# FrankBoesing/Minimal-SDR

Hardware: AMD Instinct MI355X
Metric: Msamples/s through IF->I/Q->FIR->demod->IIR chain; achieved HBM GB/s vs peak (higher is better)
Workload: dtype f32 (fp32 accumulate; matrix-core operands as 2 x fp16 pieces: int16 samples exact, taps 22 bits)

## Files before the change

### include/msdr.h

```cpp
#ifndef MSDR_H
#define MSDR_H

#include <stddef.h>
#include <stdint.h>

#ifdef __cplusplus
extern "C" {
#endif

#define MSDR_VERSION_MAJOR 0
#define MSDR_VERSION_MINOR 1

typedef int16_t q15_t;
typedef float float32_t;

typedef enum {
    MSDR_STATUS_SUCCESS        = 0,
    MSDR_STATUS_ARGUMENT_ERROR = -1,
    MSDR_STATUS_LENGTH_ERROR   = -2,
    MSDR_STATUS_SIZE_MISMATCH  = -3,
    MSDR_STATUS_NO_DEVICE      = -100,
    MSDR_STATUS_HIP_ERROR      = -101,
    MSDR_STATUS_OUT_OF_MEMORY  = -102
} msdr_status;
// ... 233 lines not shown
#define MSDR_FLAVOUR_SSB_UNITS    0x0001u
#define MSDR_FLAVOUR_ENV_UNITS    0x0002u
#define MSDR_FLAVOUR_SSB_FOLD     0x0004u
#define MSDR_FLAVOUR_ENV_FOLD     0x0008u
#define MSDR_FLAVOUR_FULL_RATE    0x0010u
#define MSDR_FLAVOUR_COMPACT      0x0020u
#define MSDR_FLAVOUR_SHARED_IQ    0x0040u
#define MSDR_FLAVOUR_AMTR         0x0080u
#define MSDR_FLAVOUR_BLOCK        0x0100u
#define MSDR_FLAVOUR_VALU_FOLD    0x0200u
#define MSDR_FLAVOUR_SEQ_CASCADE  0x0400u
#define MSDR_FLAVOUR_SEGMENTED    0x0800u
#define MSDR_FLAVOUR_FOLD_PERIOD_SHIFT 12
#define MSDR_FLAVOUR_FOLD_PERIOD(f) (((f) >> MSDR_FLAVOUR_FOLD_PERIOD_SHIFT) & 7u)
enum { MSDR_FLAVOUR_TAPS_PC = 0x8000u };
enum { MSDR_FLAVOUR_CASCADE_PC = 0x10000u };
enum { MSDR_FLAVOUR_OSC_PC = 0x20000u };
enum { MSDR_FLAVOUR_SHARED_IF = 0x40000u };
enum { MSDR_FLAVOUR_NCO_PC = 0x80000u };
enum { MSDR_FLAVOUR_DECIMATED = 0x100000u };
enum { MSDR_FLAVOUR_METER = 0x200000u };
enum { MSDR_FLAVOUR_IQ_OUT = 0x400000u };
int msdr_chain_get_info(msdr_chain *chain, msdr_chain_info *info);
const char *msdr_chain_node_kernel(msdr_chain *chain);
const char *msdr_biquad_q15_last_kernel(msdr_biquad_q15 *S);
const char *msdr_frontend_last_kernel(msdr_frontend *fe);
int msdr_chain_get_fir_history(msdr_chain *chain, uint32_t channel, int16_t *hist, uint32_t capacity, uint32_t *hist_len);
int msdr_chain_get_cmsis_state(msdr_chain *chain, uint32_t channel, float32_t *pState);
int msdr_chain_enable_timing(msdr_chain *chain, int on);
int msdr_chain_get_kernel_time(msdr_chain *chain, double *total_ms, uint64_t *launches, int reset);


typedef struct msdr_chain_graph msdr_chain_graph;
int msdr_chain_graph_create(msdr_chain *chain, uint32_t ticks, const int16_t *const *d_if, void *const *d_audio, uint64_t n_samples, msdr_chain_graph **out);
int msdr_chain_graph_launch(msdr_chain_graph *graph);
int msdr_chain_graph_destroy(msdr_chain_graph *graph);

#ifdef __cplusplus
}
#endif
#endif
```

### minimal-sdr_amd/csrc/msdr_api.hip

```cpp
#include <dlfcn.h>
#include "../../include/msdr.h"
#include "msdr_kernels.hiph"
#include "msdr_chain_fold.hiph"
#include <type_traits>
#include "msdr_chain_mfma.hiph"
#include "msdr_chain_mfw.hiph"
#include "msdr_frontend.hiph"
#include "msdr_spectrum.hiph"
#include "msdr_chain_q15mf.hiph"
#include "msdr_fir_f32mf.hiph"
#include "msdr_fir_f32tr.hiph"
#include "msdr_fir_f32tq.hiph"
#include "msdr_chain_amtr.hiph"
#include "msdr_chain_mfb.hiph"
#include "msdr_chain_q15mb.hiph"
#include "msdr_chain_q15pc.hiph"
#include "msdr_chain_f32pc.hiph"
#include "msdr_chain_oscpc.hiph"
#include "msdr_block.h"
#include "msdr_nco.h"
#include "msdr_design.h"
#include "msdr_cascade_state.h"
#include "msdr_kstack.h"
#include "msdr_sparse24.h"
// ... 2175 lines not shown
    float in_scale;
    uint32_t nstages;
    uint32_t nnodes;
    uint32_t time_segments, warmup_cfg;
    double pole_radius;
    void *d_taps, *d_osc;
    int *d_mode, *d_tapset;
    int16_t *d_hist[2];
    int cur;
    long long phase;
    BiquadCascadeTables<kChainR> *d_bq;
    float *d_bq_state;
    int fold_P;
    int mf_P;
    bool fold_fs4_exact;
    float *d_ftaps;
    int *d_fset;
    BiquadCascadeTables<kFoldR> *d_bq_fold;
    std::vector<int> h_mode, h_tapset;
    bool mf_ok;
    int mf_halo, mf_bsteps, mf_stride;
    int mf_xsteps = 0;
    int mf_merged[2] = {0, 0};
    char *d_mf_tab;
    BiquadCascadeTables<kMfL> *d_bq_mf;
    BiquadCascadeTables<32> *d_bq_mf32;
    uint32_t flags;
    int mfw_nw, mfw_waves_per_cu;
    char *d_at_tab; int at_ns, at_stride, at_nw;
    bool mf_compact, mf_share_iq;
    bool mf_fr;
    float *d_bq_state_alt;
    float *d_mw_iir;
    bool mfw_ssb_fold, mfw_am_fold;
    int mfw_am_rowlocal;
    uint32_t units_wgs_ssb;
    long long part_nseg[2], part_seg_len[2];
    long long units_tiles;
    int *d_units;
    size_t units_cap;
    uint64_t mode_gen, units_mode_gen;
    long long units_nseg;
    uint32_t units_wgs;
    int *d_btiles = nullptr;
    size_t btiles_cap = 0;
    uint64_t btiles_mode_gen = 0;
// ... 770 lines not shown
            }
        }
        if (ok && bsteps > 0) {
            const int stride = kMfHdrBytes + (bsteps + xsteps) * 2048;
            std::vector<char> blob((size_t)stride * tabs.size(), 0);
            for (size_t t = 0; t < tabs.size(); t++) {
                memcpy(blob.data() + t * stride, &tabs[t].h, sizeof(MfmaTableHeader));
                memcpy(blob.data() + t * stride + kMfHdrBytes, tabs[t].frags.data(), tabs[t].frags.size() * sizeof(_Float16));
            }
            rc = upload(ctx, blob, &c->d_mf_tab);
            if (!rc) {
                std::vector<BiquadCascadeTables<kMfL>> bt(1);
                make_cascade_tables<kMfL>(cfg->biquad_coeffs, (int)c->nstages, &bt[0]);
                rc = upload(ctx, bt, &c->d_bq_mf);
            }
            if (!rc) {
                std::vector<BiquadCascadeTables<32>> bt(1);
                make_cascade_tables<32>(cfg->biquad_coeffs, (int)c->nstages, &bt[0]);
                rc = upload(ctx, bt, &c->d_bq_mf32);
            }
            if (!rc) {
                c->mf_ok = true; c->mf_halo = H; c->mf_bsteps = bsteps; c->mf_stride = stride; c->mf_compact = compact;
                c->mf_xsteps = xsteps; c->mf_merged[0] = merged_min[0]; c->mf_merged[1] = merged_min[1];
                int best = 0, best_eff = 0, wcap = 16;
#ifdef MSDR_STAMPS
                if (const char *e = getenv("MSDR_DBG_NW")) wcap = std::max(1, std::min(16, atoi(e)));
#endif
                for (int w = 1; w <= wcap; w++) {
                    const size_t l = mw_lds_bytes(H, bsteps + xsteps, w, fr);
                    if (l > 160 * 1024) break;
                    const int wgs = std::min<int>((int)((160 * 1024) / l), wcap / w);
                    const int on_cu = wgs * w, eff = on_cu >= 4 ? 4 * (on_cu / 4) : on_cu;
                    if (eff > best_eff) { best_eff = eff; best = on_cu; c->mfw_nw = w; }
                }
                if (const char *e = getenv("MSDR_MFW_NW")) {
                    const int w = atoi(e);
                    if (w >= 1 && w <= 16 && mw_lds_bytes(H, bsteps + xsteps, w, fr) <= 160 * 1024) { c->mfw_nw = w; best = w * std::max<int>(1, std::min<int>((int)((160 * 1024) / mw_lds_bytes(H, bsteps + xsteps, w, fr)), 16 / w)); }
                }
                c->mfw_waves_per_cu = best;
                if (best > 0) rc = dzalloc(ctx, (size_t)c->channels * kBqStateFloats, &c->d_bq_state_alt);
                if (!rc && iirfold && !iirc.empty()) rc = upload(ctx, iirc, &c->d_mw_iir);
                c->mfw_ssb_fold = iirfold && !compact && c->d_mw_iir; c->mfw_am_fold = amfold && c->d_mw_iir;
                c->mfw_am_rowlocal = c->mfw_am_fold ? am_rowlocal : 0;
                if (best <= 0) c->mf_ok = false;
                if (fr && c->mfw_nw < 2) c->mf_ok = false;
            }
// ... 462 lines not shown
            const long long rounds = (nch * ns + slots - 1) / slots;
            const double cost = (double)rounds * (double)(st + (ns > 1 ? t.warm_tiles : 0));
            if (cost < best * 0.999) { best = cost; ns_ = ns; }
        }
    } else {
        long long min_seg_tiles = std::max<long long>(4, 32 * t.warm_tiles);
        long long max_nseg = std::max<long long>(1, t.tiles / min_seg_tiles);
        long long want = c->time_segments > 1 ? c->time_segments : std::max<long long>(1, (2048 + nch - 1) / nch);
        ns_ = std::max<long long>(1, std::min(want, max_nseg));
    }
    const long long st = (t.tiles + ns_ - 1) / ns_;
    return (t.tiles + st - 1) / st;
}

struct ChainLaunch {
    const char *kname;
    unsigned grid, block;
    size_t lds_bytes;
    long long nseg;
    int tile;
    uint32_t flavour;
    uint32_t env_scan;
    int merged_steps;
    const char *node_kname;
};

static int chain_fset_of(const msdr_chain *c, uint32_t ch)
{
    const int m = c->h_mode[ch];
    return c->h_tapset[ch] * 3 + (m == MSDR_MODE_LSB ? 0 : m == MSDR_MODE_USB ? 1 : 2);
}

static int chain_mfw_units(msdr_chain *c, const ChainTiles &t)
{
    if (c->units_mode_gen == c->mode_gen && c->units_tiles == t.tiles) return 0;
    const int nw = c->mfw_nw;
    std::vector<uint32_t> order(c->channels);
    for (uint32_t i = 0; i < c->channels; i++) order[i] = i;
    auto fset_of = [&](uint32_t ch) { return chain_fset_of(c, ch); };
    auto env_of = [&](uint32_t ch) { return fset_of(ch) % 3 == 2 ? 1 : 0; };
    auto key_of = [&](uint32_t ch) { return env_of(ch) * 1000000 + fset_of(ch); };
    std::stable_sort(order.begin(), order.end(), [&](uint32_t a, uint32_t b) { return key_of(a) < key_of(b); });
    long long count[2] = {0, 0};
    for (uint32_t ch : order) count[env_of(ch)]++;
    for (int part = 0; part < 2; part++) {
        c->part_nseg[part] = chain_choose_nseg(c, t, count[part]);
        c->part_seg_len[part] = ((t.tiles + c->part_nseg[part] - 1) / c->part_nseg[part]) * t.tile;
    }
    std::vector<int> units;
    units.reserve(((size_t)c->channels * std::max(c->part_nseg[0], c->part_nseg[1]) + 3 * MSDR_MAX_TAPSETS * nw) * 2);
    size_t ssb_units = 0;
    for (size_t i = 0; i < order.size(); i++) {
        if (i > 0 && fset_of(order[i]) != fset_of(order[i - 1]))
            while ((units.size() / 2) % nw) { units.push_back(-1); units.push_back(0); }
        if (env_of(order[i]) && (i == 0 || !env_of(order[i - 1]))) ssb_units = units.size() / 2;
        for (long long sg = 0; sg < c->part_nseg[env_of(order[i])]; sg++) { units.push_back((int)order[i]); units.push_back((int)sg); }
    }
    while ((units.size() / 2) % nw) { units.push_back(-1); units.push_back(0); }
    if (order.empty() || !env_of(order.back())) ssb_units = units.size() / 2;
    if (int rc = grow_device(c->ctx, &c->d_units, &c->units_cap, units.size())) return rc;
    HIP_TRY(hipMemcpyAsync(c->d_units, units.data(), units.size() * sizeof(int), hipMemcpyHostToDevice, c->ctx->stream));
    HIP_TRY(hipStreamSynchronize(c->ctx->stream));
    c->units_mode_gen = c->mode_gen; c->units_tiles = t.tiles; c->units_wgs = (uint32_t)(units.size() / 2 / nw);
    c->units_wgs_ssb = (uint32_t)(ssb_units / nw);
    return 0;
}

// ... 40 lines not shown
            oh.tab[oh.n] = o.d_tab; oh.sw[oh.n] = -o.elapsed; oh.stride[oh.n] = o.stride; oh.n++;
        }
        if (!c->d_osc_hist) HIP_TRY(hipMalloc((void **)&c->d_osc_hist, sizeof(OscHistory)));
        HIP_TRY(hipMemcpyAsync(c->d_osc_hist, &oh, sizeof oh, hipMemcpyHostToDevice, c->ctx->stream));
        HIP_TRY(hipStreamSynchronize(c->ctx->stream));
        p.osc_hist = c->d_osc_hist;
    }
    if (d.i16 == kI16InKernel && path_mfw(d.path)) p.dbg |= kChainOutI16;
    if (d.i16 == kI16ViaScratch) {
        if (int rc = grow_device(c->ctx, &c->d_f32_scratch, &c->f32_scratch_floats, (size_t)c->channels * (n_samples / c->decim))) return rc;
        p.out = c->d_f32_scratch;
    }
    p.mf_tab = c->d_mf_tab; p.mf_stride = c->mf_stride; p.mf_halo = c->mf_halo; p.mf_bsteps = c->mf_bsteps; p.mf_xsteps = c->mf_xsteps; p.bq_mf = c->d_bq_mf; p.bq_mf32 = c->d_bq_mf32;
    const int osc_P = d.mf ? c->mf_P : c->fold_P;
    p.ftaps = c->d_ftaps; p.chan_fset = c->d_fset; p.fold_period = osc_P; p.bq_fold = c->d_bq_fold;
    p.fold_rot = osc_P ? (int)(c->phase % osc_P) : 0;

    r.nseg = chain_choose_nseg(c, t, c->channels);
    const long long seg_tiles = (t.tiles + r.nseg - 1) / r.nseg;
    p.nseg = (int)r.nseg; p.seg_len = seg_tiles * t.tile; p.warm = (int)(r.nseg > 1 ? t.warm_tiles * t.tile : 0);
    r.kname = ""; r.node_kname = "";
    r.grid = (unsigned)(c->channels * r.nseg); r.block = kThreads; r.tile = t.tile;
    r.lds_bytes = t.mfw ? mw_lds_bytes(c->mf_halo, c->mf_bsteps + c->mf_xsteps, c->mfw_nw, c->mf_fr) : d.path == kPathFold ? fold_lds_bytes(p.ntaps_pad) : chain_lds_bytes(p.ntaps_pad);
    r.flavour = 0; r.env_scan = 0; r.merged_steps = -1;

    switch (d.path) {
    case kPathMfb:
        if (int rc = chain_block_tiles(c, (int)n_samples, [&](uint32_t ch) { return chain_fset_of(c, ch) % 3 == 2 ? 1 : 0; }, [&](uint32_t ch) { return chain_fset_of(c, ch); },
                                       [&](int w, int tpw) { return mb_lds_bytes(c->mf_halo, (int)n_samples, c->mf_bsteps, w, tpw); })) return rc;
        r.nseg = 1; p.nseg = 1; p.warm = 0;
        p.bq_state_out = c->d_bq_state_alt; p.mw_iir = c->d_mw_iir;
        break;
    case kPathQ15Mb:
        if (int rc = chain_block_tiles(c, (int)n_samples, [&](uint32_t ch) { const int m = c->h_mode[ch]; return (m == MSDR_MODE_LSB || m == MSDR_MODE_USB) ? 0 : 1; },
                                       [&](uint32_t ch) { return c->h_tapset[ch]; },
                                       [&](int w, int tpw) { return qb_lds_bytes(c->qm_halo, (int)n_samples, c->qm_bsteps, w, tpw); },
                                       chain_nodes_fusable(c, n_samples) ? 3 : 0)) return rc;
        r.nseg = 1; p.nseg = 1; p.warm = 0;
        for (int part = 0; part < 2 && d.nodes_fused; part++) {
            const msdr_chain::BlockPart &bp = c->bpart[part];
            if (bp.wgs && (bp.tpw != 1 || bp.nw < 3 || qb_nodes_lds_bytes(c->qm_halo, 128, c->qm_bsteps, (int)bp.nw) > 160 * 1024)) d.nodes_fused = false;
        }
        break;
    case kPathMfw:
        if (int rc = chain_mfw_units(c, t)) return rc;
        r.nseg = (c->units_wgs_ssb > 0) ? c->part_nseg[0] : c->part_nseg[1];
        p.warm = (int)(r.nseg > 1 ? t.warm_tiles * t.tile : 0);
// ... 124 lines not shown
    r.block = (unsigned)c->mfw_nw * 64;
    for (int part = 0; part < 2; part++) {
        const unsigned g = part == 0 ? c->units_wgs_ssb : c->units_wgs - c->units_wgs_ssb;
        if (g == 0) continue;
        ChainParams q = p;
        q.mf_units = c->d_units + (size_t)(part == 0 ? 0 : c->units_wgs_ssb) * c->mfw_nw * 2;
        q.nseg = (int)c->part_nseg[part]; q.seg_len = c->part_seg_len[part]; q.warm = (int)(c->part_nseg[part] > 1 ? t.warm_tiles * t.tile : 0);
        const bool fold = part == 0 ? c->mfw_ssb_fold : c->mfw_am_fold;
        const int rowlocal = (part == 1 && fold && !c->mf_fr && !c->d_at_tab) ? c->mfw_am_rowlocal : 0;
        if (part == 1 && fold && !c->d_at_tab) r.env_scan = 1u + (uint32_t)rowlocal;
        r.flavour |= part == 0 ? MSDR_FLAVOUR_SSB_UNITS : MSDR_FLAVOUR_ENV_UNITS;
        if (c->part_nseg[part] > 1) r.flavour |= MSDR_FLAVOUR_SEGMENTED;
        if (part == 1 && c->d_at_tab) {
            ChainParams a = q;
            const long long entries = (long long)g * c->mfw_nw;
            a.mf_tab = c->d_at_tab; a.mf_stride = c->at_stride; a.mf_nw = c->at_nw; a.fold_rot = (int)entries;
            const unsigned ag = (unsigned)((entries + c->at_nw - 1) / c->at_nw);
            const size_t alds = at_lds_bytes(c->at_ns, c->at_nw);
            (void)launch_chain_amtr(c->ctx->stream, c->at_ns, (int)c->nstages, ag, (unsigned)c->at_nw * 64, alds, a);
            if (int rc2 = launch_check("chain_amtr_kernel")) return rc2;
            r.flavour |= MSDR_FLAVOUR_AMTR;
            continue;
        }
        (void)launch_chain_mfw(c->ctx->stream, (int)c->nstages, part == 1, fold, c->mf_fr, rowlocal, g, r.block, r.lds_bytes, q);
        const int part_merged = mw_merges_steps((int)c->nstages, part == 1, fold, c->mf_fr, rowlocal) ? c->mf_merged[part] : 0;
        r.merged_steps = r.merged_steps < 0 ? part_merged : std::min(r.merged_steps, part_merged);
        if (int rc = launch_check("chain_mfw_kernel")) return rc;
        if (fold) r.flavour |= part == 0 ? MSDR_FLAVOUR_SSB_FOLD : MSDR_FLAVOUR_ENV_FOLD;
        if (c->mf_fr) r.flavour |= MSDR_FLAVOUR_FULL_RATE | (c->mf_compact ? MSDR_FLAVOUR_COMPACT : 0u) | ((part == 1 && c->mf_share_iq) ? MSDR_FLAVOUR_SHARED_IQ : 0u);
    }
    static const char *const names[5] = {"chain_mfw_kernel<0>", "chain_mfw_kernel<1>", "chain_mfw_kernel<2>", "chain_mfw_kernel<3>", "chain_mfw_kernel<4>"};
    static const char *const names_fr[5] = {"chain_mfw_kernel<0> full-rate NCO streams", "chain_mfw_kernel<1> full-rate NCO streams", "chain_mfw_kernel<2> full-rate NCO streams",
                                            "chain_mfw_kernel<3> full-rate NCO streams", "chain_mfw_kernel<4> full-rate NCO streams"};
    r.kname = c->mf_fr ? names_fr[c->nstages] : names[c->nstages];
    if (c->d_at_tab && c->units_wgs > c->units_wgs_ssb) r.kname = c->units_wgs_ssb ? "chain_mfw_kernel + chain_amtr_kernel" : "chain_amtr_kernel";
    std::swap(c->d_bq_state, c->d_bq_state_alt);
#ifdef MSDR_STAMPS
    if (getenv("MSDR_STAMP_PRINT")) {
        HIP_TRY(hipStreamSynchronize(c->ctx->stream));
        std::vector<unsigned long long> h((size_t)r.grid * c->mfw_nw * 8);
        HIP_TRY(hipMemcpy(h.data(), p.dbg_buf, h.size() * 8, hipMemcpyDeviceToHost));
        double sum[8] = {0}; size_t cnt = 0;
        for (size_t u = 0; u < h.size() / 8; u++) { if (!h[u * 8 + 0] && !h[u * 8 + 1]) continue; cnt++; for (int k = 0; k < 8; k++) sum[k] += (double)h[u * 8 + k]; }
        const double tl = (double)((p.n + kMwTile - 1) / kMwTile) * c->channels / std::max<size_t>(cnt, 1);
        fprintf(stderr, "stamps (cycles per tile per wave, %zu units, %.1f tiles each): prefetch-issue %.0f | mfma %.0f | demod+swap %.0f | iir %.0f | store %.0f | halo %.0f | vmwait %.0f | stage %.0f\n",
                cnt, tl, sum[0] / cnt / tl, sum[1] / cnt / tl, sum[2] / cnt / tl, sum[3] / cnt / tl, sum[4] / cnt / tl, sum[5] / cnt / tl, sum[6] / cnt / tl, sum[7] / cnt / tl);
    }
// ... 249 lines not shown
        if (int rc2 = launch_check("history_rows_kernel")) return rc2;
    } else {
        hipLaunchKernelGGL((history_kernel<int16_t>), dim3(grid_1d((long long)c->channels * c->hist_len)), dim3(256), 0, c->ctx->stream,
                           d_if, (const int16_t *)c->d_hist[c->cur], c->d_hist[c->cur ^ 1], (long long)n_samples, (int)c->hist_len,
                           (int)c->channels);
        if (int rc2 = launch_check("history_kernel")) return rc2;
    }
    c->cur ^= 1; c->gen++;
    c->phase = (c->phase + (long long)(n_samples % c->osc_len)) % c->osc_len;
    c->nco_T += n_samples; c->hist_clear = false;
    if (c->force_generic) {
        for (auto &o : c->osc_pending) o.elapsed += (long long)n_samples;
        if (c->osc_pending.empty() || c->osc_pending.back().elapsed >= (long long)c->hist_len)
            if (int rc2 = chain_leave_generic(c)) return rc2;
    }

    const char *bq_name = !c->seq_bq ? "" : c->seq_bq->per_channel ? " + biquad_df1_seq_pc_kernel" : c->seq_bq->sequential ? " + biquad_df1_seq_kernel" : " + biquad_df1_kernel";
    snprintf(c->info.kernel, sizeof c->info.kernel, "%.*s%s", (int)(sizeof c->info.kernel - 1 - strlen(bq_name)), r.kname, bq_name);
    c->info.grid = r.grid; c->info.block = r.block; c->info.lds_bytes = (uint32_t)r.lds_bytes;
    c->info.env_scan = r.env_scan; c->info.flavour = f32 ? r.flavour : 0u;
    c->info.time_segments = (uint32_t)r.nseg; c->info.warmup = (uint32_t)p.warm; c->info.tile = (uint32_t)r.tile;
    c->info.taps_padded = path_per_channel(d.path) ? (uint32_t)c->pc_np : c->ntaps_pad;
    c->info.mfma_ksteps = d.mf ? (uint32_t)(c->mf_bsteps - std::max(r.merged_steps, 0)) : path_qm(d.path) ? (uint32_t)c->qm_bsteps : 0u;
    return 0;
}

struct msdr_chain_graph {
    msdr_chain *c;
    hipGraph_t graph;
    hipGraphExec_t exec;
    uint32_t ticks;
    uint64_t n;
    const void *k_hist, *k_state, *k_tab, *k_tiles;
    int k_cur;
    uint64_t k_mode_gen;
    uint64_t k_rebuild_gen;
    const void *k_mode, *k_osc;
    bool k_taps_pc;
    bool k_nodes_pc;
    bool k_osc_pc;
    uint64_t k_osc_gen;
    bool k_block_pc;
    uint64_t k_block_epoch, k_anr_gen;
    bool k_block_q15;
    uint64_t k_block_q15_epoch;
    uint64_t k_in_row_epoch;
// ... 282 lines not shown
        chain_free(n);
        return fail(MSDR_STATUS_SIZE_MISMATCH, "internal: a live update changed the chain's geometry");
    }
    if (n->hist_len == c->hist_len) { std::swap(n->d_hist[0], c->d_hist[0]); std::swap(n->d_hist[1], c->d_hist[1]); n->cur = c->cur; }
    else {
        hipLaunchKernelGGL(hist_resize_kernel, dim3(grid_1d((long long)n->channels * n->hist_len)), dim3(256), 0, c->ctx->stream,
                           (const int16_t *)c->d_hist[c->cur], n->d_hist[n->cur], (int)n->channels, (int)c->hist_len, (int)n->hist_len);
        if (int rc2 = launch_check("hist_resize_kernel")) { chain_free(n); return rc2; }
        if (hipStreamSynchronize(c->ctx->stream) != hipSuccess) { chain_free(n); return fail(MSDR_STATUS_HIP_ERROR, "hist_resize_kernel failed"); }
    }
    n->phase = c->phase;
    if (n->d_bq_state && c->d_bq_state) std::swap(n->d_bq_state, c->d_bq_state);
    if (n->seq_bq && c->seq_bq) std::swap(n->seq_bq, c->seq_bq);
    for (int k = 0; k < 2; k++) if (n->nodes[k] && c->nodes[k]) std::swap(n->nodes[k], c->nodes[k]);
    std::swap(n->pll, c->pll); std::swap(n->d_pll_q, c->d_pll_q); std::swap(n->pll_q_cap, c->pll_q_cap);
    std::swap(n->anr, c->anr); std::swap(n->d_anr_on, c->d_anr_on); n->anr_all = c->anr_all;
    n->h_anr = c->h_anr; n->anr_gen = c->anr_gen; n->f32_pll = c->f32_pll;
    std::swap(n->d_post_pll_state, c->d_post_pll_state); std::swap(n->d_post_anr_state, c->d_post_anr_state);
    std::swap(n->post_bq, c->post_bq); n->h_post_ch = c->h_post_ch; c->h_post_ch.clear();
    n->post_mode_gen = 0; n->post_anr_gen = 0;
    n->gen = c->gen; n->dh_cache = c->dh_cache; n->dh_gen = c->dh_gen;
    n->floor_d = used_d; n->floor_sig = used_sig; n->floor_gen = c->gen;
    n->timing = c->timing; n->events.swap(c->events); n->timed_ms = c->timed_ms; n->timed_launches = c->timed_launches;
    n->info = c->info;
    n->osc_pending.swap(c->osc_pending); n->force_generic = c->force_generic;
    n->rebuild_gen = c->rebuild_gen + 1;
    n->pc_active = c->pc_active; n->pc_np = c->pc_np; std::swap(n->d_pc_taps, c->d_pc_taps); n->h_pc_taps.swap(c->h_pc_taps); n->h_pc_own.swap(c->h_pc_own);
    std::swap(n->d_pcf_taps, c->d_pcf_taps); n->h_pcf_taps.swap(c->h_pcf_taps); n->seq_forced = c->seq_forced;
    n->opc_active = c->opc_active; std::swap(n->d_osc_bank, c->d_osc_bank); n->osc_gen = c->osc_gen;
    n->block_pc = c->block_pc; n->block_epoch = c->block_epoch;
    n->block_q15 = c->block_q15; n->block_q15_epoch = c->block_q15_epoch;
    n->n_inputs = c->n_inputs; std::swap(n->d_in_row, c->d_in_row); n->in_row_epoch = c->in_row_epoch;
    n->d_meter = c->d_meter; std::swap(n->d_meter_part, c->d_meter_part); n->meter_part_cap = c->meter_part_cap; n->meter_epoch = c->meter_epoch;
    n->nco_active = c->nco_active; std::swap(n->d_nco_bank, c->d_nco_bank); std::swap(n->d_nco_tab, c->d_nco_tab);
    n->h_nco_base.swap(c->h_nco_base); n->h_nco_step.swap(c->h_nco_step); n->nco_T = c->nco_T; n->hist_clear = c->hist_clear;
    n->decim = c->decim;
    n->d_iq = c->d_iq; n->iq_pitch = c->iq_pitch;
    std::swap(*c, *n);
    if (steal_osc) { *steal_osc = n->d_osc; n->d_osc = nullptr; }
    chain_free(n);
    if (c->pc_active) {
        for (uint32_t ch = 0; ch < c->channels; ch++) if (!c->h_pc_own[ch]) chain_pc_row_shared(c, ch);
        if (int rc2 = chain_pc_upload(c, 0, c->channels)) return rc2;
    }
    return 0;
}

// ... 643 lines not shown
    }
    if (!c->anr) if (int rc = msdr_anr_create(c->ctx, c->channels, &c->anr)) return rc;
    HIP_TRY(hipStreamSynchronize(c->ctx->stream));
    hipFree(c->d_anr_on); c->d_anr_on = nullptr;
    c->anr_all = anr_on_all;
    c->anr_gen++;
    if (anr_on) {
        std::vector<int> h(anr_on, anr_on + c->channels);
        if (int rc = upload(c->ctx, h, &c->d_anr_on)) return rc;
    }
    return 0;
}

extern "C" int msdr_chain_destroy(msdr_chain *c)
{
    if (!c) return 0;
    if (int rc = bind(c->ctx)) return rc;
    (void)hipStreamSynchronize(c->ctx->stream);
    chain_free(c);
    return 0;
}

extern "C" const char *msdr_chain_node_kernel(msdr_chain *c) { return c ? c->node_kernel : nullptr; }
extern "C" int msdr_chain_get_info(msdr_chain *c, msdr_chain_info *info)
{
    if (!c || !info) return fail(MSDR_STATUS_ARGUMENT_ERROR, "null argument");
    *info = c->info;
    return 0;
}

extern "C" int msdr_chain_get_fir_history(msdr_chain *c, uint32_t channel, int16_t *hist, uint32_t capacity, uint32_t *hist_len)
{
    if (!c || channel >= c->channels) return fail(MSDR_STATUS_ARGUMENT_ERROR, "bad argument");
    if (int rc = bind(c->ctx)) return rc;
    if (hist_len) *hist_len = c->hist_len;
    if (!hist) return 0;
    if (capacity < c->hist_len) return fail(MSDR_STATUS_ARGUMENT_ERROR, "the history holds %u samples, room for %u given", c->hist_len, capacity);
    HIP_TRY(hipStreamSynchronize(c->ctx->stream));
    HIP_TRY(hipMemcpy(hist, c->d_hist[c->cur] + (size_t)channel * c->hist_len, (size_t)c->hist_len * sizeof(int16_t), hipMemcpyDeviceToHost));
    return 0;
}
extern "C" int msdr_chain_get_cmsis_state(msdr_chain *c, uint32_t channel, float32_t *pState)
{
    if (!c || !pState || channel >= c->channels) return fail(MSDR_STATUS_ARGUMENT_ERROR, "bad argument");
    if (c->arith != MSDR_ARITH_F32 || !c->seq_bq) return fail(MSDR_STATUS_ARGUMENT_ERROR, "the chain's cascade does not run behind the kernel: no pState of its own");
    return msdr_biquad_df1_f32_get_cmsis_state(c->seq_bq, channel, pState);
// ... 27 lines not shown
```

### minimal-sdr_amd/csrc/msdr_block.h

```cpp
#pragma once
#include <hip/hip_runtime.h>
#include "msdr_shared.h"
#include "msdr_pc_geometry.h"

namespace msdr {
hipError_t launch_chain_mfb(hipStream_t stream, int stages, bool am, unsigned grid, unsigned block, size_t lds_bytes, const ChainParams &p);
hipError_t launch_chain_q15mb(hipStream_t stream, int flavour, bool nodes, unsigned grid, unsigned block, size_t lds_bytes, const ChainParams &p);
hipError_t launch_chain_mfw(hipStream_t stream, int stages, bool am, bool fold, bool full_rate, int rowlocal, unsigned grid, unsigned block, size_t lds_bytes, const ChainParams &p);
hipError_t launch_chain_amtr(hipStream_t stream, int ns, int stages, unsigned grid, unsigned block, size_t lds_bytes, const ChainParams &p);
hipError_t launch_chain_fold(hipStream_t stream, int period, unsigned grid, size_t lds_bytes, const ChainParams &p);
hipError_t launch_chain_generic(hipStream_t stream, bool q15, unsigned grid, size_t lds_bytes, const ChainParams &p);
hipError_t launch_chain_q15mf(hipStream_t stream, int flavour, bool full_rate, unsigned grid, unsigned block, size_t lds_bytes, const ChainParams &p);
struct TqParams;
hipError_t launch_fir_f32tq(hipStream_t stream, int ns, bool skip1, unsigned grid, size_t lds_bytes, const TqParams &q);
hipError_t launch_fir_f32mf(hipStream_t stream, unsigned grid, unsigned block, size_t lds_bytes, const float *x, float *y, const float *hist, const char *tab,
                            long long n, int channels, int nseg, long long seg_len, int hist_len, int halo, int nsteps, int nw);
constexpr int kQ15Mult = 0, kQ15Add = 1, kQ15Sub = 2, kQ15Copy = 3;
hipError_t launch_q15_elementwise(hipStream_t stream, int op, int max_grid, const short *a, long long a_stride, const short *b, long long b_stride,
                                  short *dst, long long rows, int cols, const char **kernel);
hipError_t launch_biquad_teensy_pc(hipStream_t stream, int nodes, short *data, int *defs0, int *defs1, int channels, long long n);
hipError_t launch_chain_q15pc(hipStream_t stream, bool fir_only, int num_cus, PcParams p, PcLaunch *geo);
hipError_t launch_chain_f32pc(hipStream_t stream, bool fir_only, int num_cus, int time_segments, PcfParams p, PcLaunch *geo);
hipError_t launch_chain_q15pco(hipStream_t stream, int num_cus, PcParams p, PcLaunch *geo);
hipError_t launch_chain_f32pco(hipStream_t stream, int num_cus, int time_segments, PcfParams p, PcLaunch *geo);
int chain_pcn_max_taps(bool f32);
hipError_t launch_chain_q15pcn(hipStream_t stream, int num_cus, PcnParams p, PcLaunch *geo);
hipError_t launch_chain_f32pcn(hipStream_t stream, int num_cus, int time_segments, PcfnParams p, PcLaunch *geo);
bool chain_dec_fits(bool f32, int np, int D);
int chain_dec_max(bool f32);
int chain_dec_max_taps(bool f32, int D);
hipError_t launch_chain_q15pcnd(hipStream_t stream, int num_cus, PcndParams p, PcLaunch *geo);
// ... 12 lines not shown
```

### minimal-sdr_amd/csrc/msdr_chain_stream.hip

```cpp
#include <type_traits>
#include "msdr_kernels.hiph"
#include "msdr_chain_fold.hiph"
#include "msdr_chain_mfma.hiph"
#include "msdr_chain_mfw.hiph"
#include "msdr_chain_q15mf.hiph"
#include "msdr_fir_f32mf.hiph"
#include "msdr_fir_f32tr.hiph"
#include "msdr_chain_amtr.hiph"
#include "msdr_block.h"

namespace msdr {

hipError_t launch_chain_mfw(hipStream_t stream, int stages, bool am, bool fold, bool fr, int rowlocal, unsigned grid, unsigned block, size_t lds, const ChainParams &q)
{
    if (rowlocal) {
        if (stages != 2 || !am || !fold || fr || rowlocal > 2) return hipErrorInvalidValue;
        if (rowlocal == 1) hipLaunchKernelGGL((chain_mfw_rowlocal_kernel<1>), dim3(grid), dim3(block), lds, stream, q);
        else hipLaunchKernelGGL((chain_mfw_rowlocal_kernel<2>), dim3(grid), dim3(block), lds, stream, q);
        return hipGetLastError();
    }
#define MSDR_MFW_LAUNCH(SS, AMF, FO) do { if (fr) hipLaunchKernelGGL((chain_mfw_kernel<SS, AMF, FO, true>), dim3(grid), dim3(block), lds, stream, q); \
                                          else hipLaunchKernelGGL((chain_mfw_kernel<SS, AMF, FO, false>), dim3(grid), dim3(block), lds, stream, q); } while (0)
#define MSDR_MFW_PLAIN(SS) do { if (!am) MSDR_MFW_LAUNCH(SS, false, false); else MSDR_MFW_LAUNCH(SS, true, false); } while (0)
#define MSDR_MFW_FOLDS(SS) do { if (!fold) MSDR_MFW_PLAIN(SS); else if (!am) MSDR_MFW_LAUNCH(SS, false, true); else MSDR_MFW_LAUNCH(SS, true, true); } while (0)
    switch (stages) {
    case 0: MSDR_MFW_PLAIN(0); break;
    case 1: MSDR_MFW_FOLDS(1); break;
    case 2: MSDR_MFW_FOLDS(2); break;
    case 3: MSDR_MFW_PLAIN(3); break;
    default: MSDR_MFW_PLAIN(4); break;
    }
#undef MSDR_MFW_FOLDS
#undef MSDR_MFW_PLAIN
#undef MSDR_MFW_LAUNCH
    return hipGetLastError();
}

// ... 47 lines not shown
```

### minimal-sdr_amd/python/msdr.py

```python
import ctypes as C
import os

import numpy as np

_HERE = os.path.dirname(os.path.abspath(__file__))
LIB_PATH = os.path.join(os.path.dirname(_HERE), "lib", "libmsdr.so")

MODE_SYNCAM, MODE_AM, MODE_LSB, MODE_USB, MODE_CW = 0, 1, 2, 3, 4
SQRT_F32, SQRT_Q31 = 0, 1
MIXER_FS4, MIXER_NCO = 0, 1
ARITH_Q15, ARITH_F32 = 0, 1
BQ_LOWPASS, BQ_HIGHPASS, BQ_BANDPASS, BQ_NOTCH, BQ_LOWSHELF, BQ_HIGHSHELF = range(6)
AUDIO_SAMPLE_RATE_EXACT = 44117.64706
MAX_TAPSETS = 8
CHAIN_NO_TAP_FOLDING = 1
CHAIN_NO_MFMA = 8
CHAIN_SYNCAM_PLL = 32
CHAIN_FOLD_ANY_PERIOD = 64
CHAIN_OUT_I16 = 128
FLAVOUR_SSB_UNITS, FLAVOUR_ENV_UNITS, FLAVOUR_SSB_FOLD, FLAVOUR_ENV_FOLD = 0x1, 0x2, 0x4, 0x8
FLAVOUR_FULL_RATE, FLAVOUR_COMPACT, FLAVOUR_SHARED_IQ, FLAVOUR_AMTR = 0x10, 0x20, 0x40, 0x80
FLAVOUR_BLOCK, FLAVOUR_VALU_FOLD, FLAVOUR_SEQ_CASCADE, FLAVOUR_SEGMENTED = 0x100, 0x200, 0x400, 0x800
FLAVOUR_FOLD_PERIOD_SHIFT = 12
FLAVOUR_TAPS_PC = 0x8000
# ... 59 lines not shown
        _lib.msdr_biquad_df1_f32_set_coeffs.argtypes = [_p, _p]
        _lib.msdr_biquad_df1_f32_get_cmsis_state.argtypes = [_p, C.c_uint32, _p]
        _lib.msdr_fir_q15_set_coeffs.argtypes = [_p, _p]
        _lib.msdr_fir_f32_set_coeffs.argtypes = [_p, _p]
        _lib.msdr_chain_set_taps.argtypes = [_p, C.c_uint32, _p, _p]
        _lib.msdr_chain_set_osc.argtypes = [_p, _p, _p]
        _lib.msdr_chain_set_node_coefficients.argtypes = [_p, C.c_uint32, C.c_uint32, _p]
        for n, sig in (("msdr_chain_set_node_coefficients_channels", [_p, C.c_uint32, C.c_uint32, C.c_uint32, C.c_uint32, _p]),
                       ("msdr_biquad_q15_set_coefficients_channels", [_p, C.c_uint32, C.c_uint32, C.c_uint32, _p]),
                       ("msdr_chain_set_taps_channels", [_p, C.c_uint32, C.c_uint32, _p, _p]),
                       ("msdr_fir_q15_set_coeffs_channels", [_p, C.c_uint32, C.c_uint32, _p]),
                       ("msdr_chain_set_taps_channels_f32", [_p, C.c_uint32, C.c_uint32, _p, _p]),
                       ("msdr_fir_f32_set_coeffs_channels", [_p, C.c_uint32, C.c_uint32, _p]),
                       ("msdr_chain_set_biquad_coeffs_channels", [_p, C.c_uint32, C.c_uint32, _p]),
                       ("msdr_biquad_df1_f32_set_coeffs_channels", [_p, C.c_uint32, C.c_uint32, _p]),
                       ("msdr_chain_set_osc_channels", [_p, C.c_uint32, C.c_uint32, _p, _p]),
                       ("msdr_chain_set_block_kernel", [_p, C.c_int]),
                       ("msdr_chain_set_block_kernel_q15", [_p, C.c_int]),
                       ("msdr_chain_set_input_rows", [_p, C.c_uint32, _p]),
                       ("msdr_chain_set_nco_channels", [_p, C.c_uint32, C.c_uint32, _p, _p]),
                       ("msdr_chain_get_nco", [_p, C.c_uint32, _p, _p]),
                       ("msdr_chain_set_decimation", [_p, C.c_uint32]),
                       ("msdr_chain_get_decimation", [_p, _p]),
                       ("msdr_chain_set_meter", [_p, _p]),
                       ("msdr_chain_get_meter", [_p, _p]),
                       ("msdr_meter_dbfs", [C.c_double, C.c_uint64, C.c_double]),
                       ("msdr_chain_set_iq_out", [_p, _p, C.c_uint64]),
                       ("msdr_chain_get_iq_out", [_p, _p, _p]),
                       ("msdr_nco_step", [C.c_double, C.c_double]),
                       ("msdr_nco_table", [_p]),
                       ("msdr_nco_q15", [_p, C.c_size_t, _p, _p]),
                       ("msdr_chain_get_fir_history", [_p, C.c_uint32, _p, C.c_uint32, _p]),
                       ("msdr_chain_get_cmsis_state", [_p, C.c_uint32, _p])):
            if hasattr(_lib, n):
                getattr(_lib, n).argtypes = sig
        if hasattr(_lib, "msdr_meter_dbfs"):
            _lib.msdr_meter_dbfs.restype = C.c_double
        if hasattr(_lib, "msdr_nco_step"):
            _lib.msdr_nco_step.restype = C.c_uint32
            _lib.msdr_nco_table.restype = None
            _lib.msdr_nco_q15.restype = None
        _lib.msdr_chain_set_biquad_coeffs.argtypes = [_p, _p]
        _lib.msdr_malloc.argtypes = [_p, C.c_size_t, _p]
        _lib.msdr_free.argtypes = [_p, _p]
        _lib.msdr_memcpy_h2d.argtypes = [_p, _p, _p, C.c_size_t]
        _lib.msdr_memcpy_d2h.argtypes = [_p, _p, _p, C.c_size_t]
# ... 785 lines not shown
        _ck(self.ctx.lib.msdr_chain_set_node_coefficients_channels(self.h, C.c_uint32(node), C.c_uint32(first_channel), C.c_uint32(c.shape[0]),
                                                                   C.c_uint32(stage), _hp(c)))

    def set_biquad_coeffs(self, coeffs):
        c = np.ascontiguousarray(coeffs, np.float32).reshape(-1)
        if self.stages and c.size != 5 * self.stages:
            raise ValueError("set_biquad_coeffs: %d values given, the chain's cascade has %d stages x 5" % (c.size, self.stages))
        _ck(self.ctx.lib.msdr_chain_set_biquad_coeffs(self.h, _hp(c)))

    def set_biquad_coeffs_channels(self, first_channel, coeffs):
        c = _cascade_per_channel("set_biquad_coeffs_channels", coeffs, self.stages)
        _ck(self.ctx.lib.msdr_chain_set_biquad_coeffs_channels(self.h, C.c_uint32(first_channel), C.c_uint32(c.shape[0]), _hp(c)))

    def node_kernel(self):
        return _kernel_name(self.ctx.lib.msdr_chain_node_kernel, self.h)

    def info(self):
        i = ChainInfo()
        _ck(self.ctx.lib.msdr_chain_get_info(self.h, C.byref(i)))
        return {"kernel": i.kernel.decode(), "grid": i.grid, "block": i.block, "lds_bytes": i.lds_bytes,
                "time_segments": i.time_segments, "warmup": i.warmup, "tile": i.tile, "taps_padded": i.taps_padded,
                "mfma_ksteps": i.mfma_ksteps, "env_scan": i.env_scan, "flavour": i.flavour}

    def enable_timing(self, on=True):
        _ck(self.ctx.lib.msdr_chain_enable_timing(self.h, int(on)))

    def kernel_time(self, reset=True):
        ms, n = C.c_double(0), C.c_uint64(0)
        _ck(self.ctx.lib.msdr_chain_get_kernel_time(self.h, C.byref(ms), C.byref(n), int(reset)))
        return ms.value, n.value


GATHER_SLOTS = 4


def comm_unique_id():
    buf = C.create_string_buffer(128)
    _ck(load_library().msdr_comm_get_unique_id(buf))
    return buf.raw


class Comm:

    def __init__(self, ctx, unique_id, rank, world):
        self.ctx, self.rank, self.world = ctx, rank, world
        h = _p()
# ... 22 lines not shown
```

Baseline: 531,200.

## Dispatch geometry-specialised MFW chain kernels when all partition tap tables share a shape

```diff
diff --git a/include/msdr.h b/include/msdr.h
--- a/include/msdr.h
+++ b/include/msdr.h
@@ -279,6 +279,7 @@
 enum { MSDR_FLAVOUR_METER = 0x200000u };
 enum { MSDR_FLAVOUR_IQ_OUT = 0x400000u };
 int msdr_chain_get_info(msdr_chain *chain, msdr_chain_info *info);
+int msdr_chain_get_geometry(msdr_chain *chain, uint32_t *id);
 const char *msdr_chain_node_kernel(msdr_chain *chain);
 const char *msdr_biquad_q15_last_kernel(msdr_biquad_q15 *S);
 const char *msdr_frontend_last_kernel(msdr_frontend *fe);
diff --git a/minimal-sdr_amd/csrc/msdr_api.hip b/minimal-sdr_amd/csrc/msdr_api.hip
--- a/minimal-sdr_amd/csrc/msdr_api.hip
+++ b/minimal-sdr_amd/csrc/msdr_api.hip
@@ -2221,6 +2221,9 @@
     int mf_halo, mf_bsteps, mf_stride;
     int mf_xsteps = 0;
     int mf_merged[2] = {0, 0};
+    std::vector<uint8_t> mf_tab_geom;
+    std::vector<int> part_fsets[2];
+    uint32_t last_geom = 0;
     char *d_mf_tab;
     BiquadCascadeTables<kMfL> *d_bq_mf;
     BiquadCascadeTables<32> *d_bq_mf32;
@@ -3037,6 +3040,11 @@
             if (!rc) {
                 c->mf_ok = true; c->mf_halo = H; c->mf_bsteps = bsteps; c->mf_stride = stride; c->mf_compact = compact;
                 c->mf_xsteps = xsteps; c->mf_merged[0] = merged_min[0]; c->mf_merged[1] = merged_min[1];
+                static_assert(kMwMergedBytes == kSp24Bytes, "MwGeom places the merged steps as the table builder does");
+                bool geom_on = true;
+                if (const char *e = getenv("MSDR_MFW_GEOM")) geom_on = atoi(e) != 0;
+                c->mf_tab_geom.clear();
+                if (geom_on && !fr) for (const Tab &T : tabs) c->mf_tab_geom.push_back((uint8_t)mw_geom_of(T.h, H));
                 int best = 0, best_eff = 0, wcap = 16;
 #ifdef MSDR_STAMPS
                 if (const char *e = getenv("MSDR_DBG_NW")) wcap = std::max(1, std::min(16, atoi(e)));
@@ -3545,6 +3553,7 @@
     uint32_t flavour;
     uint32_t env_scan;
     int merged_steps;
+    uint32_t geom;
     const char *node_kname;
 };
 
@@ -3566,6 +3575,8 @@
     std::stable_sort(order.begin(), order.end(), [&](uint32_t a, uint32_t b) { return key_of(a) < key_of(b); });
     long long count[2] = {0, 0};
     for (uint32_t ch : order) count[env_of(ch)]++;
+    c->part_fsets[0].clear(); c->part_fsets[1].clear();
+    for (uint32_t ch : order) { std::vector<int> &f = c->part_fsets[env_of(ch)]; if (f.empty() || f.back() != fset_of(ch)) f.push_back(fset_of(ch)); }
     for (int part = 0; part < 2; part++) {
         c->part_nseg[part] = chain_choose_nseg(c, t, count[part]);
         c->part_seg_len[part] = ((t.tiles + c->part_nseg[part] - 1) / c->part_nseg[part]) * t.tile;
@@ -3652,7 +3663,7 @@
     r.kname = ""; r.node_kname = "";
     r.grid = (unsigned)(c->channels * r.nseg); r.block = kThreads; r.tile = t.tile;
     r.lds_bytes = t.mfw ? mw_lds_bytes(c->mf_halo, c->mf_bsteps + c->mf_xsteps, c->mfw_nw, c->mf_fr) : d.path == kPathFold ? fold_lds_bytes(p.ntaps_pad) : chain_lds_bytes(p.ntaps_pad);
-    r.flavour = 0; r.env_scan = 0; r.merged_steps = -1;
+    r.flavour = 0; r.env_scan = 0; r.merged_steps = -1; r.geom = 0;
 
     switch (d.path) {
     case kPathMfb:
@@ -3823,7 +3834,18 @@
             r.flavour |= MSDR_FLAVOUR_AMTR;
             continue;
         }
-        (void)launch_chain_mfw(c->ctx->stream, (int)c->nstages, part == 1, fold, c->mf_fr, rowlocal, g, r.block, r.lds_bytes, q);
+        int geom = 0;
+        if (mw_geom_flavour((int)c->nstages, part == 1, fold, c->mf_fr, rowlocal) && !c->mf_tab_geom.empty()) {
+            const int P = std::max(q.fold_period, 1);
+            for (size_t k = 0; k < c->part_fsets[part].size(); k++) {
+                const size_t ti = (size_t)c->part_fsets[part][k] * P + q.fold_rot;
+                const int id = ti < c->mf_tab_geom.size() ? c->mf_tab_geom[ti] : 0;
+                geom = (k == 0 || id == geom) ? id : 0;
+                if (!geom) break;
+            }
+        }
+        r.geom = std::max(r.geom, (uint32_t)geom);
+        (void)launch_chain_mfw(c->ctx->stream, (int)c->nstages, part == 1, fold, c->mf_fr, rowlocal, g, r.block, r.lds_bytes, q, geom);
         const int part_merged = mw_merges_steps((int)c->nstages, part == 1, fold, c->mf_fr, rowlocal) ? c->mf_merged[part] : 0;
         r.merged_steps = r.merged_steps < 0 ? part_merged : std::min(r.merged_steps, part_merged);
         if (int rc = launch_check("chain_mfw_kernel")) return rc;
@@ -4119,6 +4141,7 @@
     c->info.time_segments = (uint32_t)r.nseg; c->info.warmup = (uint32_t)p.warm; c->info.tile = (uint32_t)r.tile;
     c->info.taps_padded = path_per_channel(d.path) ? (uint32_t)c->pc_np : c->ntaps_pad;
     c->info.mfma_ksteps = d.mf ? (uint32_t)(c->mf_bsteps - std::max(r.merged_steps, 0)) : path_qm(d.path) ? (uint32_t)c->qm_bsteps : 0u;
+    c->last_geom = r.geom;
     return 0;
 }
 
@@ -4447,7 +4470,7 @@
     n->gen = c->gen; n->dh_cache = c->dh_cache; n->dh_gen = c->dh_gen;
     n->floor_d = used_d; n->floor_sig = used_sig; n->floor_gen = c->gen;
     n->timing = c->timing; n->events.swap(c->events); n->timed_ms = c->timed_ms; n->timed_launches = c->timed_launches;
-    n->info = c->info;
+    n->info = c->info; n->last_geom = c->last_geom;
     n->osc_pending.swap(c->osc_pending); n->force_generic = c->force_generic;
     n->rebuild_gen = c->rebuild_gen + 1;
     n->pc_active = c->pc_active; n->pc_np = c->pc_np; std::swap(n->d_pc_taps, c->d_pc_taps); n->h_pc_taps.swap(c->h_pc_taps); n->h_pc_own.swap(c->h_pc_own);
@@ -5137,6 +5160,12 @@
 }
 
 extern "C" const char *msdr_chain_node_kernel(msdr_chain *c) { return c ? c->node_kernel : nullptr; }
+extern "C" int msdr_chain_get_geometry(msdr_chain *c, uint32_t *id)
+{
+    if (!c || !id) return fail(MSDR_STATUS_ARGUMENT_ERROR, "null argument");
+    *id = c->last_geom;
+    return 0;
+}
 extern "C" int msdr_chain_get_info(msdr_chain *c, msdr_chain_info *info)
 {
     if (!c || !info) return fail(MSDR_STATUS_ARGUMENT_ERROR, "null argument");
diff --git a/minimal-sdr_amd/csrc/msdr_block.h b/minimal-sdr_amd/csrc/msdr_block.h
--- a/minimal-sdr_amd/csrc/msdr_block.h
+++ b/minimal-sdr_amd/csrc/msdr_block.h
@@ -6,7 +6,7 @@
 namespace msdr {
 hipError_t launch_chain_mfb(hipStream_t stream, int stages, bool am, unsigned grid, unsigned block, size_t lds_bytes, const ChainParams &p);
 hipError_t launch_chain_q15mb(hipStream_t stream, int flavour, bool nodes, unsigned grid, unsigned block, size_t lds_bytes, const ChainParams &p);
-hipError_t launch_chain_mfw(hipStream_t stream, int stages, bool am, bool fold, bool full_rate, int rowlocal, unsigned grid, unsigned block, size_t lds_bytes, const ChainParams &p);
+hipError_t launch_chain_mfw(hipStream_t stream, int stages, bool am, bool fold, bool full_rate, int rowlocal, unsigned grid, unsigned block, size_t lds_bytes, const ChainParams &p, int geom = 0);
 hipError_t launch_chain_amtr(hipStream_t stream, int ns, int stages, unsigned grid, unsigned block, size_t lds_bytes, const ChainParams &p);
 hipError_t launch_chain_fold(hipStream_t stream, int period, unsigned grid, size_t lds_bytes, const ChainParams &p);
 hipError_t launch_chain_generic(hipStream_t stream, bool q15, unsigned grid, size_t lds_bytes, const ChainParams &p);
diff --git a/minimal-sdr_amd/csrc/msdr_chain_stream.hip b/minimal-sdr_amd/csrc/msdr_chain_stream.hip
--- a/minimal-sdr_amd/csrc/msdr_chain_stream.hip
+++ b/minimal-sdr_amd/csrc/msdr_chain_stream.hip
@@ -11,8 +11,16 @@
 
 namespace msdr {
 
-hipError_t launch_chain_mfw(hipStream_t stream, int stages, bool am, bool fold, bool fr, int rowlocal, unsigned grid, unsigned block, size_t lds, const ChainParams &q)
+hipError_t launch_chain_mfw(hipStream_t stream, int stages, bool am, bool fold, bool fr, int rowlocal, unsigned grid, unsigned block, size_t lds, const ChainParams &q, int geom)
 {
+    if (geom) {
+        if (!mw_geom_flavour(stages, am, fold, fr, rowlocal) || rowlocal > 2 || geom > kMwGeomCount) return hipErrorInvalidValue;
+#define MSDR_MFW_GEOM_LAUNCH(G) do { if (rowlocal == 1) hipLaunchKernelGGL((chain_mfw_geom_kernel<1, G>), dim3(grid), dim3(block), lds, stream, q); \
+                              else hipLaunchKernelGGL((chain_mfw_geom_kernel<2, G>), dim3(grid), dim3(block), lds, stream, q); } while (0)
+        if (geom == MwGeomEnv256::id) MSDR_MFW_GEOM_LAUNCH(MwGeomEnv256); else MSDR_MFW_GEOM_LAUNCH(MwGeomEnv512);
+#undef MSDR_MFW_GEOM_LAUNCH
+        return hipGetLastError();
+    }
     if (rowlocal) {
         if (stages != 2 || !am || !fold || fr || rowlocal > 2) return hipErrorInvalidValue;
         if (rowlocal == 1) hipLaunchKernelGGL((chain_mfw_rowlocal_kernel<1>), dim3(grid), dim3(block), lds, stream, q);
diff --git a/minimal-sdr_amd/python/msdr.py b/minimal-sdr_amd/python/msdr.py
--- a/minimal-sdr_amd/python/msdr.py
+++ b/minimal-sdr_amd/python/msdr.py
@@ -105,6 +105,7 @@
                        ("msdr_chain_get_nco", [_p, C.c_uint32, _p, _p]),
                        ("msdr_chain_set_decimation", [_p, C.c_uint32]),
                        ("msdr_chain_get_decimation", [_p, _p]),
+                       ("msdr_chain_get_geometry", [_p, _p]),
                        ("msdr_chain_set_meter", [_p, _p]),
                        ("msdr_chain_get_meter", [_p, _p]),
                        ("msdr_meter_dbfs", [C.c_double, C.c_uint64, C.c_double]),
@@ -936,6 +937,11 @@
                 "time_segments": i.time_segments, "warmup": i.warmup, "tile": i.tile, "taps_padded": i.taps_padded,
                 "mfma_ksteps": i.mfma_ksteps, "env_scan": i.env_scan, "flavour": i.flavour}
 
+    def geometry(self):
+        g = C.c_uint32(0)
+        _ck(self.ctx.lib.msdr_chain_get_geometry(self.h, C.byref(g)))
+        return g.value
+
     def enable_timing(self, on=True):
         _ck(self.ctx.lib.msdr_chain_enable_timing(self.h, int(on)))
 
```

Result: faster. 543,700 (median of 6 runs) (+2.4%).
